# zhukovanadezhda/collaborative-filtering

Measured on AMD Instinct MI355X. Metric: ratings/sec per ALS iteration at k=64, higher is better.
Workload: dtype f32 (storage, solve, accumulate); Gram products as 2-way fp16 split (error <= 2^-23) on fp16 MFMA; rows over the condition limit redone in f64 (solve_dtype=auto)

## Files before the change

### collaborative-filtering_amd/csrc/als_device.hpp

```cpp
#pragma once
#include <hip/hip_runtime.h>
#include <stdint.h>
#include <type_traits>

typedef float f32x4 __attribute__((ext_vector_type(4)));
typedef float f32x2 __attribute__((ext_vector_type(2)));

#define ALS_EPS 1e-10f

__device__ __forceinline__ float readlane_f(float v, int src_lane) {
    return __int_as_float(__builtin_amdgcn_readlane(__float_as_int(v), src_lane));
}
__device__ __forceinline__ float bperm_f(float v, int src_lane) {
    return __int_as_float(__builtin_amdgcn_ds_bpermute(src_lane << 2, __float_as_int(v)));
}
__device__ __forceinline__ int bperm_i(int v, int src_lane) {
    return __builtin_amdgcn_ds_bpermute(src_lane << 2, v);
}
template <unsigned long long MASK>
__device__ __forceinline__ float select_lanes(float a, float b) {
    return __builtin_amdgcn_inverse_ballot_w64(MASK) ? a : b;
}
template <int BOUND, int RR>
constexpr unsigned long long lanes_below() {
    constexpr int n = BOUND - 64 * RR;
    return n <= 0 ? 0ull : (n >= 64 ? ~0ull : ((1ull << n) - 1ull));
}

__device__ __forceinline__ float wave_sum(float v) {
    auto dpp = [](float x, auto ctrl, auto rows) {
        return __int_as_float(__builtin_amdgcn_update_dpp(0, __float_as_int(x), decltype(ctrl)::value,
                                                          decltype(rows)::value, 0xf, false));
    };
    using std::integral_constant;
    v += dpp(v, integral_constant<int, 0xB1>{}, integral_constant<int, 0xf>{});
    v += dpp(v, integral_constant<int, 0x4E>{}, integral_constant<int, 0xf>{});
    v += dpp(v, integral_constant<int, 0x141>{}, integral_constant<int, 0xf>{});
    v += dpp(v, integral_constant<int, 0x140>{}, integral_constant<int, 0xf>{});
    v += dpp(v, integral_constant<int, 0x142>{}, integral_constant<int, 0xa>{});
    v += dpp(v, integral_constant<int, 0x143>{}, integral_constant<int, 0xc>{});
    return readlane_f(v, 63);
}
__device__ __forceinline__ float wave_max_nonneg(float v) {
    auto dpp = [](uint32_t x, auto ctrl, auto rows) {
        return (uint32_t)__builtin_amdgcn_update_dpp(0, (int)x, decltype(ctrl)::value, decltype(rows)::value, 0xf, false);
    };
    using std::integral_constant;
    uint32_t u = (uint32_t)__float_as_int(v);
    u = max(u, dpp(u, integral_constant<int, 0xB1>{}, integral_constant<int, 0xf>{}));
    u = max(u, dpp(u, integral_constant<int, 0x4E>{}, integral_constant<int, 0xf>{}));
    u = max(u, dpp(u, integral_constant<int, 0x141>{}, integral_constant<int, 0xf>{}));
    u = max(u, dpp(u, integral_constant<int, 0x140>{}, integral_constant<int, 0xf>{}));
    u = max(u, dpp(u, integral_constant<int, 0x142>{}, integral_constant<int, 0xa>{}));
    u = max(u, dpp(u, integral_constant<int, 0x143>{}, integral_constant<int, 0xc>{}));
    return __int_as_float(__builtin_amdgcn_readlane((int)u, 63));
}
__device__ __forceinline__ double wave_sum_d(double v) {
#pragma unroll
    for (int o = 32; o >= 1; o >>= 1) v += __shfl_xor(v, o, 64);
    return v;
}

__device__ __forceinline__ void wave_lds_sync() {
    __builtin_amdgcn_fence(__ATOMIC_SEQ_CST, "workgroup");
    __builtin_amdgcn_wave_barrier();
}

template <int KB>
__device__ __forceinline__ int perm_to_col(int p) { return KB * (p & 15) + (p >> 4); }

template <int KB>
__device__ __forceinline__ void load_frow(const float* __restrict__ p, float (&f)[KB]) {
    if constexpr (KB % 4 == 0) {
#pragma unroll
        for (int j = 0; j < KB / 4; ++j) {
            f32x4 v = *reinterpret_cast<const f32x4*>(p + 4 * j);
            f[4 * j] = v.x; f[4 * j + 1] = v.y; f[4 * j + 2] = v.z; f[4 * j + 3] = v.w;
        }
    } else if constexpr (KB % 2 == 0) {
#pragma unroll
        for (int j = 0; j < KB / 2; ++j) {
            f32x2 v = *reinterpret_cast<const f32x2*>(p + 2 * j);
            f[2 * j] = v.x; f[2 * j + 1] = v.y;
        }
    } else {
#pragma unroll
        for (int j = 0; j < KB; ++j) f[j] = p[j];
    }
}

template <int KB>
struct KCfg {
    static constexpr int KP = 16 * KB;
    static constexpr int NACC = KB * (KB + 1) / 2;
    static constexpr int NR = (KP + 63) / 64;
    static constexpr int lcol_off(int J) { return 16 * (J * KP - 8 * J * (J - 1)); }
    __device__ static __forceinline__ int lcol_off_rt(int J) { return 16 * (J * KP - 8 * J * (J - 1)); }
    static constexpr int LDS_FLOATS = lcol_off(KB);
    static_assert(lcol_off(KB) == NACC * 256, "the L image and a full accumulator set have the same size");
#ifndef ALS_WPW
#define ALS_WPW 1
#endif
    static constexpr int WPW = ALS_WPW;
#ifndef ALS_MINW_LE4
#define ALS_MINW_LE4 3
#endif
    static constexpr int MINW = (KB <= 4) ? ALS_MINW_LE4 : (KB <= 6 ? 2 : 1);
    static constexpr int SLOT_ITEMS = NACC * 4 + 2 * KB + 2;
    static constexpr int GS = (KB <= 8) ? 8 : 4;
};

template <int KP>
__device__ __forceinline__ float solve_regs(const float (&a)[KP], float di, float rb, int lane,
                                            float* y_out = nullptr) {
    int zero;
    asm volatile("s_mov_b32 %0, 0" : "=s"(zero));
    const unsigned long long ones = ~0ull;
    float rs = rb * di;
#pragma unroll
    for (int j = 0; j < KP; ++j) {
        const float yj = readlane_f(rs, j);
        const unsigned long long mask = (j >= 63) ? 0ull : (ones << (j + 1 + zero));
        const float cf = __builtin_amdgcn_inverse_ballot_w64(mask) ? a[j] * di : 0.f;
        rs = fmaf(-cf, yj, rs);
    }
    if (y_out) *y_out = rs;
    rs *= di;
#pragma unroll
    for (int i = KP - 1; i >= 0; --i) {
        const float xi = readlane_f(rs, i);
        const unsigned long long mask = (i <= 0) ? 0ull : ~(ones << (i + zero));
        const float cf = __builtin_amdgcn_inverse_ballot_w64(mask) ? a[i] * di : 0.f;
        rs = fmaf(-cf, xi, rs);
    }
    return rs;
}

template <int KB>
__device__ __forceinline__ void solve_stream_plain(const float* __restrict__ M, float (&rb)[KCfg<KB>::NR], int lane,
                                             float* y_out = nullptr) {
    constexpr int KP = KCfg<KB>::KP, NR = KCfg<KB>::NR;
    int ic[NR];
    float di[NR], rs[NR];
#pragma unroll
    for (int rr = 0; rr < NR; ++rr) {
        ic[rr] = min(lane + 64 * rr, KP - 1);
        di[rr] = M[ic[rr] * KP + ic[rr]];
        rs[rr] = rb[rr] * di[rr];
// ... 331 lines not shown
```

### collaborative-filtering_amd/csrc/gs_sweep.hip

```cpp
#include <atomic>
#include <cstdlib>
#include "als_device.hpp"
#include "als_hip.h"

extern "C" int als_gs_sweep(const als_gs_sweep_params* p, void* stream);

namespace {

template <int KB>
struct GsCfg {
    static constexpr int WPW = (KB <= 4) ? 4 : (KB <= 6 ? 2 : 1);
};

template <int KB>
__global__ __launch_bounds__(64 * GsCfg<KB>::WPW)
void k_gs_level(const als_gs_sweep_params P) {
    using C = KCfg<KB>;
    constexpr int KP = C::KP, NR = C::NR;
    constexpr int LD = KP + 1;
    constexpr int IMG = KP * LD + 3 * KP;
    __shared__ float lds_all[(KB <= 4) ? 1 : GsCfg<KB>::WPW * IMG];
    const int lane = threadIdx.x & 63;
    const int wave = threadIdx.x >> 6;
    const int64_t tid = (int64_t)blockIdx.x * GsCfg<KB>::WPW + wave;
// ... 128 lines not shown
    const int64_t i64 = item;
    const int64_t s0 = P.S_ptr[item], s1 = P.S_ptr[item + 1];
    const double* M = (const double*)P.factor + i64 * KP * KP;
    const double* rhs = (const double*)P.rhs + i64 * KP;
    const double* colsum = (const double*)P.colsum + i64 * KP;
    int ic[NR], col[NR];
    double g[NR];
#pragma unroll
    for (int rr = 0; rr < NR; ++rr) {
        ic[rr] = min(lane + 64 * rr, KP - 1);
        col[rr] = perm_to_col<KB>(ic[rr]);
        g[rr] = 0.0;
    }
    for (int64_t t = s0; t < s1; ++t) {
        const int sj = P.S_idx[t];
        const double sv = (double)P.S_val[t];
#pragma unroll
        for (int rr = 0; rr < NR; ++rr) g[rr] = fma(sv, (double)P.V[(int64_t)sj * P.ld + col[rr]], g[rr]);
    }
    double di[NR], rs[NR], rhs_i[NR], y[NR];
#pragma unroll
    for (int rr = 0; rr < NR; ++rr) {
        di[rr] = M[ic[rr] * KP + ic[rr]];
        rhs_i[rr] = rhs[ic[rr]];
        rs[rr] = (rhs_i[rr] + (double)P.alpha * g[rr]) * di[rr];
    }
    for (int j = 0; j < KP; ++j) {
        double sel = rs[0];
#pragma unroll
        for (int rr = 1; rr < NR; ++rr) sel = ((j >> 6) == rr) ? rs[rr] : sel;
        const double yj = readlane_f64(sel, j & 63);
#pragma unroll
        for (int rr = 0; rr < NR; ++rr) {
            const double cf = (lane + 64 * rr > j) ? M[j * KP + ic[rr]] * di[rr] : 0.0;
            rs[rr] = fma(-cf, yj, rs[rr]);
        }
    }
#pragma unroll
    for (int rr = 0; rr < NR; ++rr) { y[rr] = rs[rr]; rs[rr] *= di[rr]; }
    for (int i = KP - 1; i >= 0; --i) {
        double sel = rs[0];
#pragma unroll
        for (int rr = 1; rr < NR; ++rr) sel = ((i >> 6) == rr) ? rs[rr] : sel;
        const double xi = readlane_f64(sel, i & 63);
#pragma unroll
        for (int rr = 0; rr < NR; ++rr) {
            const double cf = (lane + 64 * rr < i) ? M[i * KP + ic[rr]] * di[rr] : 0.0;
            rs[rr] = fma(-cf, xi, rs[rr]);
        }
    }
    double dot = 0.0, xr = 0.0, yy = 0.0, xx = 0.0;
#pragma unroll
    for (int rr = 0; rr < NR; ++rr)
        if (lane + 64 * rr < KP) {
            const double x = rs[rr];
            P.V[i64 * P.ld + col[rr]] = (float)x;
            dot = fma(colsum[ic[rr]], x, dot); xr = fma(rhs_i[rr], x, xr);
            yy = fma(y[rr], y[rr], yy); xx = fma(x, x, xx);
        }
    dot = wave_sum_d(dot);
    const double nnz = (double)(P.indptr[item + 1] - P.indptr[item]);
    const double lb = (double)(P.lambda_bias_row ? P.lambda_bias_row[item] : P.lambda_bias_scalar);
    const double sumr = ((const double*)P.sumr)[item];
    const double bnew = (sumr - dot) / (nnz + lb + 1e-10);
    const double bold = (double)P.bias[item];
    __builtin_amdgcn_sched_barrier(0);
    if (lane == 0) P.bias[item] = (float)bnew;
    if (P.stat_out) {
        xr = wave_sum_d(xr); yy = wave_sum_d(yy); xx = wave_sum_d(xx);
        if (lane == 0) {
            const double sumr2 = ((const double*)P.sumr2)[item];
            const double s1v = sumr - nnz * bnew;
            const double s2v = sumr2 - 2.0 * bnew * sumr + nnz * bnew * bnew;
            const double cross = xr + (bold - bnew) * dot;
            const double quad = yy - (double)P.lambda_eff[item] * xx;
            P.stat_out[2 * i64] = (float)(s1v - dot);
            P.stat_out[2 * i64 + 1] = (float)(s2v - 2.0 * cross + quad);
        }
    }
}

constexpr unsigned GS_SENTINEL = 0x7fc0dea1u;

__device__ __forceinline__ float ld_agent(const float* p) {
    return __int_as_float(__hip_atomic_load(reinterpret_cast<const int*>(p), __ATOMIC_RELAXED, __HIP_MEMORY_SCOPE_AGENT));
}
__device__ __forceinline__ void st_agent(float* p, float v) {
    __hip_atomic_store(reinterpret_cast<int*>(p), __float_as_int(v), __ATOMIC_RELAXED, __HIP_MEMORY_SCOPE_AGENT);
}

#ifdef ALS_GS_STAMPS
__device__ unsigned long long g_gs_stamps[8];
#define GS_STAMP(slot) do { const unsigned long long now_ = __builtin_amdgcn_s_memtime(); st_acc[slot] += now_ - st_t; st_t = now_; } while (0)
#else
#define GS_STAMP(slot) do { } while (0)
#endif

template <int KB, bool STREAM>
struct DfCfg {
    static constexpr bool IMAGE = KB > 4 && !STREAM;
    static constexpr int WPW = IMAGE ? 1 : 4;
    static constexpr int LD = KCfg<KB>::KP + 1;
    static constexpr int IMG = IMAGE ? KCfg<KB>::KP * LD + 3 * KCfg<KB>::KP : 1;
};

template <int KB, bool STREAM>
__global__ __launch_bounds__((64 * DfCfg<KB, STREAM>::WPW), (DfCfg<KB, STREAM>::IMAGE ? 1 : 2))
void k_gs_dataflow(const als_gs_sweep_params P, const int32_t* __restrict__ Sw, float* pub,
                   int32_t* err, int64_t nitems, int nwaves, const float* __restrict__ nondep) {
    using C = KCfg<KB>;
    constexpr int KP = C::KP, NR = C::NR;
    using D = DfCfg<KB, STREAM>;
    constexpr int LD = D::LD;
    constexpr bool IMAGE = D::IMAGE;
    constexpr unsigned long long SPIN_LIMIT = 1ull << 27;
    __shared__ float lds_img[D::IMG];
    float* Al = lds_img;
    float* vec = lds_img + (IMAGE ? KP * LD : 0);
    float* dinv = vec + (IMAGE ? 2 * KP : 0);
    const int lane = threadIdx.x & 63;
    const int gw = blockIdx.x * D::WPW + (threadIdx.x >> 6);
    int ic[NR], col[NR];
#pragma unroll
    for (int rr = 0; rr < NR; ++rr) {
        ic[rr] = min(lane + 64 * rr, KP - 1);
        col[rr] = perm_to_col<KB>(ic[rr]);
    }
#ifdef ALS_GS_STAMPS
    unsigned long long st_acc[6] = {0, 0, 0, 0, 0, 0};
    unsigned long long st_t = __builtin_amdgcn_s_memtime();
#endif
    for (int64_t it = gw; it < nitems; it += nwaves) {
        const int item = P.items[it];
        const int64_t i64 = item;
        const int64_t s0 = P.S_ptr[item], s1 = P.S_ptr[item + 1];
        const float nnz = (float)(P.indptr[item + 1] - P.indptr[item]);
        const float lb = P.lambda_bias_row ? P.lambda_bias_row[item] : P.lambda_bias_scalar;
        const float* M = P.factor + i64 * KP * KP;
        constexpr int KPR = (KB <= 4) ? KP : 1;
        float a[KPR];
        float di0 = 0.f;
        if constexpr (KB <= 4) {
#pragma unroll
            for (int p = 0; p < KP; ++p) a[p] = M[p * KP + ic[0]];
            di0 = M[ic[0] * KP + ic[0]];
        } else if constexpr (IMAGE) {
            for (int p0 = 0; p0 < KP; p0 += 8) {
                float t[8][NR];
#pragma unroll
                for (int u = 0; u < 8; ++u)
#pragma unroll
                    for (int rr = 0; rr < NR; ++rr) t[u][rr] = M[(p0 + u) * KP + ic[rr]];
#pragma unroll
                for (int u = 0; u < 8; ++u)
#pragma unroll
                    for (int rr = 0; rr < NR; ++rr)
                        if (lane + 64 * rr < KP) {
                            Al[(p0 + u) * LD + ic[rr]] = t[u][rr];
                            if (ic[rr] == p0 + u) dinv[ic[rr]] = t[u][rr];
                        }
            }
        }
        float rhs_i[NR], cs_i[NR], g[NR];
#pragma unroll
        for (int rr = 0; rr < NR; ++rr) {
            rhs_i[rr] = P.rhs[i64 * KP + ic[rr]];
            cs_i[rr] = P.colsum[i64 * KP + ic[rr]];
            g[rr] = 0.f;
        }
        constexpr int GB = (NR == 1) ? 16 : 8;
#ifdef ALS_GS_STAMPS
        asm volatile("s_waitcnt vmcnt(0)" ::: "memory");
// ... 366 lines not shown
```

### collaborative-filtering_amd/csrc/row_solve.hip

```cpp
#include <type_traits>
#include "als_device.hpp"
#include "als_hip.h"
#include "row_common.hpp"

namespace {

template <int KB>
struct RowAcc {
    f32x4 acc[KCfg<KB>::NACC];
    float rhs[KB];
    float cs[KB];
    float sumr;
    float sumr2;
    __device__ __forceinline__ void zero() {
#pragma unroll
        for (int a = 0; a < KCfg<KB>::NACC; ++a) acc[a] = f32x4{0.f, 0.f, 0.f, 0.f};
#pragma unroll
        for (int b = 0; b < KB; ++b) { rhs[b] = 0.f; cs[b] = 0.f; }
        sumr = 0.f; sumr2 = 0.f;
    }
};

template <int KB, bool FULL>
__device__ __forceinline__ void process_chunk(RowAcc<KB>& A, int off_l, float r_l, int nvalid,
// ... 181 lines not shown
    const int c = lane & 15, q = lane >> 4;
    const float* Fc = F + KB * c;
    int nflush = 0;
    f32x4 E[MODE == 2 ? KB : 1];
    const uint32_t* Pc = planes + KB * c;
    const int sel_c = (c == 0) ? 0x05040100 : (c == 2) ? 0x07060302 : 0x0c0c0c0c;
    const int ones_c = (c == 1) ? 0x3C003C00 : 0;
    const float inv_s = __int_as_float((254 - ((__float_as_int(S) >> 23) & 0xff)) << 23);
    if constexpr (MODE == 2) {
#pragma unroll
        for (int b = 0; b < KB; ++b) E[b] = f32x4{0.f, 0.f, 0.f, 0.f};
    }
    int idx1 = (lane < len) ? __builtin_nontemporal_load(idxp + lane) : zero_row;
    int idx2 = (64 + lane < len) ? __builtin_nontemporal_load(idxp + 64 + lane) : zero_row;
    float val1 = (lane < len) ? __builtin_nontemporal_load(valp + lane) : 0.f;
    float bo1 = (lane < len) ? bias_other[idx1] : 0.f;
    for (int base = 0; base < len; base += 64) {
        const int idx0 = idx1;
        const float val0 = val1, bo0 = bo1;
        idx1 = idx2;
        const int t2 = base + 128 + lane;
        idx2 = (t2 < len) ? __builtin_nontemporal_load(idxp + t2) : zero_row;
        const int t1 = base + 64 + lane;
        val1 = (t1 < len) ? __builtin_nontemporal_load(valp + t1) : 0.f;
        bo1 = (t1 < len) ? bias_other[idx1] : 0.f;
        const int nvalid = min(64, len - base);
        const bool ok = lane < nvalid;
        const float rb = val0 - mu - bo0;
        A.sumr += ok ? rb : 0.f;
        A.sumr2 = ok ? fmaf(rb, rb, A.sumr2) : A.sumr2;
        const float r0 = ok ? (rb - bself) : 0.f;
        const int off0 = idx0 * ld;
        if constexpr (MODE == 0) {
            if (nvalid == 64) process_chunk<KB, true>(A, off0, r0, 64, Fc, q);
            else              process_chunk<KB, false>(A, off0, r0, nvalid, Fc, q);
        } else {
            if constexpr (MODE == 2) {
                const _Float16 rh = (_Float16)r0;
                const _Float16 rl = (_Float16)(r0 - (float)rh);
                const int rp = (int)__builtin_bit_cast(unsigned short, rh) | ((int)__builtin_bit_cast(unsigned short, rl) << 16);
                if (nvalid == 64) process_chunk_planes<KB, true>(A, E, off0, rp, 64, Pc, q, sel_c, ones_c);
                else              process_chunk_planes<KB, false>(A, E, off0, rp, nvalid, Pc, q, sel_c, ones_c);
            } else {
                if (nvalid == 64) process_chunk_f16x2<KB, true>(A, off0, r0, 64, Fc, q, S);
                else              process_chunk_f16x2<KB, false>(A, off0, r0, nvalid, Fc, q, S);
            }
            if (((base >> 6) + 1) % (FLUSH_GROUPS / 2) == 0 && base + 64 < len) {
                mfma_results_settle();
                if constexpr (MODE == 2) fold_planes_rhs<KB>(A, E, q, inv_s);
                flush_acc<KB>(A, Ls, lane, nflush == 0);
                ++nflush;
            }
        }
    }
    if (MODE != 0) mfma_results_settle();
    if constexpr (MODE == 2) fold_planes_rhs<KB>(A, E, q, inv_s);
    if (MODE != 0 && nflush > 0) {
        unflush_acc<KB>(A, Ls, lane);
        wave_lds_sync();
    }
}

template <int KB>
__device__ __forceinline__ void store_partial(const RowAcc<KB>& A, float* __restrict__ ws, int lane) {
    int it = 0;
#pragma unroll
    for (int a = 0; a < KCfg<KB>::NACC; ++a)
#pragma unroll
        for (int r = 0; r < 4; ++r) ws[(it++) * 64 + lane] = A.acc[a][r];
#pragma unroll
    for (int b = 0; b < KB; ++b) ws[(it++) * 64 + lane] = A.rhs[b];
#pragma unroll
    for (int b = 0; b < KB; ++b) ws[(it++) * 64 + lane] = A.cs[b];
    ws[(it++) * 64 + lane] = A.sumr;
    ws[it * 64 + lane] = A.sumr2;
}

template <int KB>
__device__ __forceinline__ void add_partial(RowAcc<KB>& A, const float* __restrict__ ws, int lane) {
    int it = 0;
#pragma unroll
    for (int a = 0; a < KCfg<KB>::NACC; ++a)
#pragma unroll
        for (int r = 0; r < 4; ++r) A.acc[a][r] += ws[(it++) * 64 + lane];
#pragma unroll
    for (int b = 0; b < KB; ++b) A.rhs[b] += ws[(it++) * 64 + lane];
#pragma unroll
    for (int b = 0; b < KB; ++b) A.cs[b] += ws[(it++) * 64 + lane];
    A.sumr += ws[(it++) * 64 + lane];
    A.sumr2 += ws[it * 64 + lane];
}

template <int KB, int J, int T, bool SOLVE>
__device__ __forceinline__ void panel_pivot(float (&p)[KCfg<KB>::NR][16], Chol<KB>& S, int lane) {
    constexpr int NR = KCfg<KB>::NR;
    constexpr int PIV = 16 * J + T, RP = PIV >> 6, LP = PIV & 63;
    constexpr int DR = (16 * J) >> 6, DL = (16 * J) & 63;
    const float prep = bperm_f(p[DR][T], DL + (lane & 15));
    const float d = readlane_f(p[RP][T], LP);
    const float inv = __builtin_amdgcn_rsqf(d);
    float l[NR];
#pragma unroll
    for (int rr = 0; rr < NR; ++rr) { l[rr] = p[rr][T] * inv; p[rr][T] = l[rr]; }
    float lrep = -(prep * inv);
    asm("s_nop 1" : "+v"(lrep));
    float yt = 0.f;
    if constexpr (SOLVE) yt = readlane_f(S.b[RP], LP) * inv;
    panel_trailing<KB, T + 1>(p, l, lrep);
    if constexpr (SOLVE) {
#pragma unroll
        for (int rr = 0; rr < NR; ++rr) S.b[rr] = fmaf(-l[rr], yt, S.b[rr]);
        S.y[RP] = select_lanes<1ull << LP>(yt, S.y[RP]);
    }
}

template <int KB, int J, int T, bool SOLVE>
__device__ __forceinline__ void panel_pivots(float (&p)[KCfg<KB>::NR][16], Chol<KB>& S, int lane) {
    if constexpr (T < 16) {
        panel_pivot<KB, J, T, SOLVE>(p, S, lane);
        panel_pivots<KB, J, T + 1, SOLVE>(p, S, lane);
    }
}

template <int KB, int J, bool SOLVE>
__device__ __forceinline__ void chol_panel(RowAcc<KB>& A, Chol<KB>& S, float* __restrict__ Ls, int lane) {
    using C = KCfg<KB>;
    constexpr int KP = C::KP, NR = C::NR;
    constexpr int OFF = C::lcol_off(J);
    const int c = lane & 15, q = lane >> 4;
    {
        const int swzc = (((c >> 2) ^ q) << 2) + (c & 3);
#pragma unroll
        for (int I = J; I < KB; ++I)
#pragma unroll
            for (int r = 0; r < 4; ++r)
                Ls[OFF + (16 * (I - J) + 4 * q + r) * 16 + swzc] = A.acc[blk_idx(I, J)][r];
    }
    wave_lds_sync();
    float p[NR][16];
    const int si = (lane >> 2) & 3;
#pragma unroll
    for (int rr = 0; rr < NR; ++rr) {
        const int i = lane + 64 * rr;
        const int rowi = min(max(i, 16 * J), KP - 1) - 16 * J;
#pragma unroll
        for (int g = 0; g < 4; ++g) {
            const f32x4 v = *reinterpret_cast<const f32x4*>(Ls + OFF + rowi * 16 + ((g ^ si) << 2));
            p[rr][4 * g] = v.x; p[rr][4 * g + 1] = v.y; p[rr][4 * g + 2] = v.z; p[rr][4 * g + 3] = v.w;
        }
    }
    wave_lds_sync();
    panel_pivots<KB, J, 0, SOLVE>(p, S, lane);
#pragma unroll
    for (int rr = 0; rr < NR; ++rr) {
        const int i = lane + 64 * rr;
        if (i >= 16 * J && i < KP) {
#pragma unroll
            for (int g = 0; g < 4; ++g) {
                const f32x4 v = {p[rr][4 * g], p[rr][4 * g + 1], p[rr][4 * g + 2], p[rr][4 * g + 3]};
                *reinterpret_cast<f32x4*>(Ls + OFF + (i - 16 * J) * 16 + ((g ^ si) << 2)) = v;
            }
        }
    }
    wave_lds_sync();
    {
        constexpr int DR = (16 * J) >> 6, DL = (16 * J) & 63;
        const float dl = Ls[OFF + c * 16 + (c & 3)];
        S.di[DR] = select_lanes<0xFFFFull << DL>(__builtin_amdgcn_rcpf(dl), S.di[DR]);
    }
    if constexpr (J + 1 < KB) {
        f32x4 op[KB - J - 1];
        const int sg = ((q ^ ((c >> 2) & 3)) << 2);
#pragma unroll
// ... 170 lines not shown
        chol_panels<KB, 0, true>(A, S, Ls, lane);
        const bool spd = chol_spd<KB>(S, lane);
        if (P.cond_limit > 0.f) {
            if (row_needs_f64<KB>(S, P, row, spd, mean_eig, short_row_bound, lane)) return;
        } else if (!spd && lane == 0) atomicMax(P.status, row + 1);
    }
    float x[NR];
    if (!(P.reserved0 & 4)) backward_solve<KB>(Ls, S, x, lane);
    else {
#pragma unroll
        for (int rr = 0; rr < NR; ++rr) x[rr] = S.y[rr];
    }

    float dot = 0.f, xr = 0.f, yy = 0.f, xx = 0.f;
#pragma unroll
    for (int rr = 0; rr < NR; ++rr) {
        if (lane + 64 * rr < KP) {
            dot = fmaf(csrow[rr], x[rr], dot);
            xr = fmaf(rhs0[rr], x[rr], xr);
            yy = fmaf(S.y[rr], S.y[rr], yy);
            xx = fmaf(x[rr], x[rr], xx);
        }
    }
    dot = wave_sum(dot);
    const float nnz = (float)(P.indptr[row + 1] - P.indptr[row]);
    const float lb = P.lambda_bias_row ? P.lambda_bias_row[row] : P.lambda_bias_scalar;
    const float bnew = (sumr - dot) / (nnz + lb + ALS_EPS);
    const float bold = P.bias_self[row];
    float st1 = 0.f, st2 = 0.f;
    if (P.stat_out) {
        xr = wave_sum(xr); yy = wave_sum(yy); xx = wave_sum(xx);
        const double bn = bnew, dt = dot;
        const double s1 = (double)sumr - (double)nnz * bn;
        const double s2 = (double)sumr2 - 2.0 * bn * (double)sumr + (double)nnz * bn * bn;
        const double cross = (double)xr + ((double)bold - bn) * dt;
        const double quad = (double)yy - (double)lam * (double)xx;
        const double sd2 = s2 - 2.0 * cross + quad;
        if (P.cond_limit > 0.f && !(sd2 >= 1e-3 * s2)) {
            if (lane == 0) P.redo_rows[atomicAdd(P.redo_count, 1)] = row;
            return;
        }
        st1 = (float)(s1 - dt);
        st2 = (float)sd2;
    }
#pragma unroll
    for (int rr = 0; rr < NR; ++rr)
        if (lane + 64 * rr < KP) P.X_out[r64 * P.ld + colrow[rr]] = x[rr];
    __builtin_amdgcn_sched_barrier(0);
    if (lane == 0) {
        P.bias_out[row] = bnew;
        if (P.stat_out) { P.stat_out[2 * r64] = st1; P.stat_out[2 * r64 + 1] = st2; }
    }
}

template <int KB, int MODE>
__global__ __launch_bounds__(64 * KCfg<KB>::WPW, KCfg<KB>::MINW)
void k_row_tasks(const als_row_solve_params P) {
    using C = KCfg<KB>;
    __shared__ __attribute__((aligned(16))) float lds_all[C::WPW * C::LDS_FLOATS];
    const int lane = threadIdx.x & 63;
    const int wave = threadIdx.x >> 6;
    const int wave_u = wave;
    const int64_t tid = (int64_t)blockIdx.x * C::WPW + wave_u;
    if (tid >= P.ntasks) return;
    const als_task t = P.tasks[tid];
    const int row = t.row;
    const int seg = t.seg;
    const int slot = t.slot;
    const int64_t rbeg = P.indptr[row], rend = P.indptr[row + 1];
    const int64_t beg = rbeg + (int64_t)seg * ALS_SPLIT_CHUNK;
    const int len = (int)min((int64_t)ALS_SPLIT_CHUNK, rend - beg);
    const float mu = (float)(*P.mu);
    const float bself = P.bias_self[row];

    const float S = (MODE != 0) ? P.F_scale[0] : 1.f;

    RowAcc<KB> A;
    A.zero();
    if (!(P.reserved0 & 1))
        gram_accumulate<KB, MODE>(A, P.indices + beg, P.vals + beg, len, P.F, P.ld, P.F_zero_row,
                                  P.bias_other, mu, bself, lane, lds_all + wave * C::LDS_FLOATS, S,
                                  (const uint32_t*)P.F_planes);
    if (slot >= 0) {
        store_partial<KB>(A, (float*)P.workspace + (size_t)slot * C::SLOT_ITEMS * 64, lane);
        return;
    }
    finish_row<KB>(A, P, row, lds_all + wave_u * C::LDS_FLOATS, lane);
}

template <int KB, int NB>
__device__ __forceinline__ void row_dual(const als_row_solve_params& P, int row, int64_t beg, int len,
                                         float* __restrict__ Ls, int lane) {
    constexpr int KP = KCfg<KB>::KP, NR = KCfg<KB>::NR, NSLAB = (KP + 31) / 32;
    constexpr int NS = KCfg<NB>::NR;
    const int c = lane & 15, q = lane >> 4;
    const float bold = P.bias_self[row];
    const float mu = (float)*P.mu;
    bool ok[NS];
    int idx_l[NS];
    float r_l[NS];
#pragma unroll
    for (int ss = 0; ss < NS; ++ss) {
        const int t = lane + 64 * ss;
        ok[ss] = t < len;
        idx_l[ss] = ok[ss] ? P.indices[beg + t] : P.F_zero_row;
        r_l[ss] = ok[ss] ? (P.vals[beg + t] - mu - P.bias_other[idx_l[ss]]) - bold : 0.f;
    }
    const int nblk = (len + 15) >> 4;
    int off[NB];
#pragma unroll
    for (int I = 0; I < NB; ++I)
        off[I] = bperm_i(idx_l[(16 * I) >> 6], (16 * I + c) & 63) * P.ld;

    const float Sc = P.F_scale[0];
    RowAcc<NB> A;
    A.zero();
    for (int s = 0; s < NSLAB; ++s) {
        const bool in = 32 * s + 8 * q < KP;
        i32x4 H[NB], L[NB];
#pragma unroll
        for (int I = 0; I < NB; ++I) {
            float f[8];
            if (I < nblk && in) {
                const f32x4 v0 = *reinterpret_cast<const f32x4*>(P.F + (uint32_t)off[I] + 32 * s + 8 * q);
                const f32x4 v1 = *reinterpret_cast<const f32x4*>(P.F + (uint32_t)off[I] + 32 * s + 8 * q + 4);
                f[0] = v0.x; f[1] = v0.y; f[2] = v0.z; f[3] = v0.w; f[4] = v1.x; f[5] = v1.y; f[6] = v1.z; f[7] = v1.w;
            } else {
#pragma unroll
                for (int e = 0; e < 8; ++e) f[e] = 0.f;
            }
#pragma unroll
            for (int e = 0; e < 8; e += 2) {
                int hw, lw;
                split2(f[e], f[e + 1], Sc, hw, lw);
                H[I][e >> 1] = hw; L[I][e >> 1] = lw;
            }
        }
#pragma unroll
        for (int bi = 0; bi < NB; ++bi)
#pragma unroll
            for (int bj = 0; bj <= bi; ++bj) {
                if (bi >= nblk) continue;
                f32x4 acc = A.acc[blk_idx(bi, bj)];
                const h16x8 hi = __builtin_bit_cast(h16x8, H[bi]), hj = __builtin_bit_cast(h16x8, H[bj]);
                const h16x8 li = __builtin_bit_cast(h16x8, L[bi]), lj = __builtin_bit_cast(h16x8, L[bj]);
                acc = __builtin_amdgcn_mfma_f32_16x16x32_f16(li, hj, acc, 0, 0, 0);
                acc = __builtin_amdgcn_mfma_f32_16x16x32_f16(hi, lj, acc, 0, 0, 0);
                acc = __builtin_amdgcn_mfma_f32_16x16x32_f16(hi, hj, acc, 0, 0, 0);
                A.acc[blk_idx(bi, bj)] = acc;
            }
    }
    mfma_results_settle();
    {
        const float un = P.F_scale[1];
#pragma unroll
        for (int a = 0; a < KCfg<NB>::NACC; ++a) A.acc[a] *= un;
    }
    const float lam = (P.lambda_row ? P.lambda_row[row] : P.lambda_scalar) + ALS_EPS;
    const float dual_mean_eig = (P.cond_limit > 0.f) ? gram_trace<NB>(A, lane) / (float)max(min(len, P.k), 1) + lam : 0.f;
#pragma unroll
    for (int J = 0; J < NB; ++J) {
        const float dv = (16 * J + c < len) ? lam : 1.0f;
#pragma unroll
        for (int r = 0; r < 4; ++r) A.acc[blk_idx(J, J)][r] += (4 * q + r == c) ? dv : 0.f;
    }
    Chol<NB> S;
#pragma unroll
    for (int ss = 0; ss < NS; ++ss) { S.b[ss] = r_l[ss]; S.di[ss] = 0.f; S.y[ss] = 0.f; }
// ... 14 lines not shown
    for (int ss = 0; ss < NS; ++ss) {
        const int lim = min(len - 64 * ss, 64);
        for (int i0 = 0; i0 < lim; i0 += 8) {
            float fv[8][NR], wi[8];
#pragma unroll
            for (int u = 0; u < 8; ++u) {
                const int i = min(i0 + u, 63);
                wi[u] = (i0 + u < lim) ? readlane_f(w[ss], i) : 0.f;
                const int o = __builtin_amdgcn_readlane(idx_l[ss], i) * P.ld;
#pragma unroll
                for (int rr = 0; rr < NR; ++rr) fv[u][rr] = P.F[(uint32_t)o + min(lane + 64 * rr, KP - 1)];
            }
#pragma unroll
            for (int u = 0; u < 8; ++u)
#pragma unroll
                for (int rr = 0; rr < NR; ++rr) x[rr] = fmaf(fv[u][rr], wi[u], x[rr]);
        }
    }
    const int64_t r64 = row;
#pragma unroll
    for (int rr = 0; rr < NR; ++rr)
        if (lane + 64 * rr < KP) P.X_out[r64 * P.ld + lane + 64 * rr] = x[rr];
    const float nnz = (float)len;
    const float lb = P.lambda_bias_row ? P.lambda_bias_row[row] : P.lambda_bias_scalar;
    float wsum = 0.f;
#pragma unroll
    for (int ss = 0; ss < NS; ++ss) wsum += ok[ss] ? w[ss] : 0.f;
    const float sw = wave_sum(wsum);
    const float bnew = (nnz * bold + lam * sw) / (nnz + lb + ALS_EPS);
    if (lane == 0) P.bias_out[row] = bnew;
    if (P.stat_out) {
        float e1 = 0.f, e2 = 0.f;
#pragma unroll
        for (int ss = 0; ss < NS; ++ss) {
            const float e = ok[ss] ? (bold - bnew) + lam * w[ss] : 0.f;
            e1 += e;
            e2 = fmaf(e, e, e2);
        }
        const float s1 = wave_sum(e1), s2 = wave_sum(e2);
        if (lane == 0) { P.stat_out[2 * r64] = s1; P.stat_out[2 * r64 + 1] = s2; }
    }
}

template <int KB>
__global__ __launch_bounds__(256, 3)
void k_row_dual(const als_row_solve_params P, int64_t task0, int64_t ntail) {
    using C4 = KCfg<4>;
    __shared__ __attribute__((aligned(16))) float lds_all[4 * C4::LDS_FLOATS];
    const int lane = threadIdx.x & 63, wave = threadIdx.x >> 6;
    const int64_t tid = (int64_t)blockIdx.x * 4 + wave;
    if (tid >= ntail) return;
    float* Ls = lds_all + wave * C4::LDS_FLOATS;
    const int row = P.tasks[task0 + tid].row;
    const int64_t beg = P.indptr[row];
    const int len = (int)(P.indptr[row + 1] - beg);
    if (len > 64 || len < 1) {
        if (lane == 0) atomicMax(P.status, row + 1);
        return;
    }
    if (len <= 16) row_dual<KB, 1>(P, row, beg, len, Ls, lane);
    else if (len <= 32) row_dual<KB, 2>(P, row, beg, len, Ls, lane);
    else if (len <= 48) row_dual<KB, 3>(P, row, beg, len, Ls, lane);
    else row_dual<KB, 4>(P, row, beg, len, Ls, lane);
}

template <int KB>
__global__ __launch_bounds__(128, 2)
void k_row_dual_mid(const als_row_solve_params P, int64_t task0, int64_t nmid) {
    using C6 = KCfg<6>;
    __shared__ __attribute__((aligned(16))) float lds_all[2 * C6::LDS_FLOATS];
    const int lane = threadIdx.x & 63, wave = threadIdx.x >> 6;
    const int64_t tid = (int64_t)blockIdx.x * 2 + wave;
    if (tid >= nmid) return;
    float* Ls = lds_all + wave * C6::LDS_FLOATS;
    const int row = P.tasks[task0 + tid].row;
    const int64_t beg = P.indptr[row];
    const int len = (int)(P.indptr[row + 1] - beg);
    if (len > 96 || len <= 64) {
        if (lane == 0) atomicMax(P.status, row + 1);
        return;
    }
    if (len <= 80) row_dual<KB, 5>(P, row, beg, len, Ls, lane);
    else row_dual<KB, 6>(P, row, beg, len, Ls, lane);
}

template <int KB>
__global__ __launch_bounds__(64 * KCfg<KB>::WPW, KCfg<KB>::MINW)
void k_row_long(const als_row_solve_params P) {
    using C = KCfg<KB>;
    __shared__ __attribute__((aligned(16))) float lds_all[C::WPW * C::LDS_FLOATS];
    const int lane = threadIdx.x & 63;
    const int wave = threadIdx.x >> 6;
    const int64_t tid = (int64_t)blockIdx.x * C::WPW + wave;
    if (tid >= P.nlong) return;
    const als_long_row lr = P.long_rows[tid];
    RowAcc<KB> A;
    A.zero();
    add_partial<KB>(A, (const float*)P.workspace + (size_t)lr.slot0 * C::SLOT_ITEMS * 64, lane);
    finish_row<KB>(A, P, lr.row, lds_all + wave * C::LDS_FLOATS, lane);
}

template <int KB>
__global__ __launch_bounds__(256)
void k_sum_slots(const als_long_row* __restrict__ long_rows, float* __restrict__ workspace) {
    constexpr int N = KCfg<KB>::SLOT_ITEMS * 64;
    const als_long_row lr = long_rows[blockIdx.x];
    const int e = blockIdx.y * 256 + threadIdx.x;
    if (e >= N || lr.nslots < 2) return;
    float* w0 = workspace + (size_t)lr.slot0 * N + e;
    float acc = 0.f + w0[0];
    for (int s = 1; s < lr.nslots; ++s) acc += w0[(size_t)s * N];
    w0[0] = acc;
}

__global__ __launch_bounds__(256)
void k_factor_scale(const float* __restrict__ F, int64_t n4, float* __restrict__ scale, int32_t* __restrict__ redo_count) {
    __shared__ uint32_t wmax[4];
    const f32x4* __restrict__ F4 = reinterpret_cast<const f32x4*>(F);
    uint32_t m = 0;
    const int64_t stride = (int64_t)gridDim.x * 256;
    for (int64_t i = (int64_t)blockIdx.x * 256 + threadIdx.x; i < n4; i += 4 * stride) {
        f32x4 v[4];
#pragma unroll
        for (int u = 0; u < 4; ++u)
            v[u] = (i + u * stride < n4) ? F4[i + u * stride] : f32x4{0.f, 0.f, 0.f, 0.f};
#pragma unroll
        for (int u = 0; u < 4; ++u)
#pragma unroll
            for (int e = 0; e < 4; ++e) m = max(m, (uint32_t)__float_as_int(v[u][e]) & 0x7FFFFFFFu);
    }
#pragma unroll
    for (int o = 32; o >= 1; o >>= 1) m = max(m, (uint32_t)__shfl_xor((int)m, o, 64));
    if ((threadIdx.x & 63) == 0) wmax[threadIdx.x >> 6] = m;
    __syncthreads();
    if (threadIdx.x == 0) {
        uint32_t* w = reinterpret_cast<uint32_t*>(scale);
        atomicMax(&w[2], max(max(wmax[0], wmax[1]), max(wmax[2], wmax[3])));
        __threadfence();
        if (atomicAdd(&w[3], 1u) == gridDim.x - 1) {
            __threadfence();
            const uint32_t mx = atomicMax(&w[2], 0u);
            const int e = (int)(mx >> 23);
            const int se = min(max(268 - e, 67), 187);
            scale[0] = __int_as_float(se << 23);
            scale[1] = __int_as_float((381 - 2 * se) << 23);
            atomicExch(&w[2], 0u);
            atomicExch(&w[3], 0u);
            if (redo_count) *redo_count = 0;
        }
    }
}

int launch_factor_scale(const float* F, int64_t nfloats, float* scale, int32_t* redo_count, hipStream_t st) {
    const int64_t n4 = nfloats / 4;
    const unsigned grid = (unsigned)min((int64_t)512, max((int64_t)1, (n4 + 1023) / 1024));
    hipLaunchKernelGGL(k_factor_scale, dim3(grid), dim3(256), 0, st, F, n4, scale, redo_count);
    return hipGetLastError() == hipSuccess ? 0 : ALS_E_LAUNCH;
}

__global__ void k_reset_word(int32_t* w) { *w = 0; }

template <int KB>
__global__ __launch_bounds__(256)
void k_split_planes(const float* __restrict__ F, int64_t npieces, const float* __restrict__ scale,
                    uint32_t* __restrict__ planes) {
    typedef uint32_t u32x4 __attribute__((ext_vector_type(4)));
    const float S = scale[0];
    for (int64_t e = (int64_t)blockIdx.x * 256 + threadIdx.x; e < npieces; e += (int64_t)gridDim.x * 256) {
        uint32_t h[KB / 2], l[KB / 2];
#pragma unroll
        for (int v4 = 0; v4 < KB / 4; ++v4) {
            const f32x4 x = reinterpret_cast<const f32x4*>(F)[e * (KB / 4) + v4];
            int h01, l01, h23, l23;
            split2(x[0], x[1], S, h01, l01);
            split2(x[2], x[3], S, h23, l23);
            h[2 * v4] = (uint32_t)h01; h[2 * v4 + 1] = (uint32_t)h23;
            l[2 * v4] = (uint32_t)l01; l[2 * v4 + 1] = (uint32_t)l23;
        }
        if constexpr (KB == 4) {
            reinterpret_cast<u32x4*>(planes)[e] = u32x4{h[0], h[1], l[0], l[1]};
        } else {
            reinterpret_cast<u32x4*>(planes)[2 * e] = u32x4{h[0], h[1], h[2], h[3]};
            reinterpret_cast<u32x4*>(planes)[2 * e + 1] = u32x4{l[0], l[1], l[2], l[3]};
        }
    }
}

template <int KB>
int launch_row_solve(const als_row_solve_params* p, hipStream_t st) {
    using C = KCfg<KB>;
    const bool plain = p->gram_mode == ALS_GRAM_F16X2 && p->reserved0 == 0 && p->X_out && p->bias_out &&
                       !p->gram_out && !p->factor_out && !p->rhs_out && !p->colsum_out && !p->sumr_out &&
                       !p->sumr2_out && !p->rhs_extra && !p->diag_extra;
    int64_t ntail = 0, nmid = 0;
    if (plain && p->ndual_tail >= 0 && p->ndual_mid >= 0 && (int64_t)p->ndual_tail + p->ndual_mid <= p->ntasks) {
        ntail = p->ndual_tail;
        if constexpr (KB >= 7) nmid = p->ndual_mid;
    }
    const int64_t nprimal = p->ntasks - ntail - nmid;
    if (nprimal > 0) {
        als_row_solve_params q = *p;
        q.ntasks = nprimal;
        const unsigned grid = (unsigned)((nprimal + C::WPW - 1) / C::WPW);
        bool planes = false;
        if constexpr (KB == 4 || KB == 8)
            planes = p->gram_mode == ALS_GRAM_F16X2 && p->F_planes != nullptr && p->reserved0 == 0;
        if (planes) {
            if constexpr (KB == 4 || KB == 8) {
                const int64_t npieces = ((int64_t)p->F_zero_row + 1) * 16;
                const unsigned sgrid = (unsigned)min((int64_t)4096, (npieces + 255) / 256);
                hipLaunchKernelGGL(k_split_planes<KB>, dim3(sgrid), dim3(256), 0, st, p->F, npieces, p->F_scale,
                                   (uint32_t*)p->F_planes);
                hipLaunchKernelGGL((k_row_tasks<KB, 2>), dim3(grid), dim3(64 * C::WPW), 0, st, q);
            }
        } else if (p->gram_mode == ALS_GRAM_F16X2)
            hipLaunchKernelGGL((k_row_tasks<KB, 1>), dim3(grid), dim3(64 * C::WPW), 0, st, q);
        else
            hipLaunchKernelGGL((k_row_tasks<KB, 0>), dim3(grid), dim3(64 * C::WPW), 0, st, q);
    }
    {
        if (ntail > 0)
            hipLaunchKernelGGL(k_row_dual<KB>, dim3((unsigned)((ntail + 3) / 4)), dim3(256), 0, st, *p, nprimal + nmid, ntail);
    }
    if constexpr (KB >= 7) {
        if (nmid > 0)
            hipLaunchKernelGGL(k_row_dual_mid<KB>, dim3((unsigned)((nmid + 1) / 2)), dim3(128), 0, st, *p, nprimal, nmid);
    }
    if (p->nlong > 0) {
        hipLaunchKernelGGL(k_sum_slots<KB>, dim3((unsigned)p->nlong, (C::SLOT_ITEMS * 64 + 255) / 256), dim3(256), 0, st,
                           p->long_rows, (float*)p->workspace);
        const unsigned grid = (unsigned)((p->nlong + C::WPW - 1) / C::WPW);
        hipLaunchKernelGGL(k_row_long<KB>, dim3(grid), dim3(64 * C::WPW), 0, st, *p);
    }
    return hipGetLastError() == hipSuccess ? 0 : ALS_E_LAUNCH;
}

}

int als_row_solve_f64_dispatch(const als_row_solve_params* p, hipStream_t st);
int als_row_redo_f64_dispatch(const als_row_solve_params* p, hipStream_t st);

extern "C" int als_version(void) { return ALS_HIP_VERSION; }
extern "C" int als_padded_k(int k) { return (k < 1 || k > ALS_MAX_K) ? ALS_E_BADK : 16 * ((k + 15) / 16); }
extern "C" int als_perm_index(int k, int c) {
    const int ld = als_padded_k(k);
    if (ld < 0 || c < 0 || c >= ld) return ALS_E_BADARG;
    const int KB = ld / 16;
    return 16 * (c % KB) + c / KB;
}
extern "C" int64_t als_partial_slot_bytes(int k) {
    const int ld = als_padded_k(k);
    if (ld < 0) return ALS_E_BADK;
    const int KB = ld / 16;
    return (int64_t)(KB * (KB + 1) / 2 * 4 + 2 * KB + 2) * 64 * sizeof(float);
}

extern "C" int als_factor_scale(const float* F, int64_t nfloats, float* scale, void* stream) {
    if (!F || !scale || nfloats < 0 || (nfloats & 3) || ((uintptr_t)F & 15)) return ALS_E_BADARG;
    return launch_factor_scale(F, nfloats, scale, nullptr, (hipStream_t)stream);
}

extern "C" int als_row_solve(const als_row_solve_params* p, void* stream) {
    if (!p) return ALS_E_BADARG;
    const int ld = als_padded_k(p->k);
    if (ld < 0) return ALS_E_BADK;
    if (p->ld != ld || !p->indptr || !p->indices || !p->vals || !p->F || !p->bias_self ||
        !p->bias_other || !p->mu || !p->status || p->ntasks < 0 || p->nlong < 0 || p->F_zero_row < 0 ||
        (p->gram_mode != ALS_GRAM_F32 && p->gram_mode != ALS_GRAM_F16X2 && p->gram_mode != ALS_GRAM_F64) ||
        (int64_t)p->F_zero_row * ld >= ((int64_t)1 << 31))
        return ALS_E_BADARG;
    if (p->ntasks > 0 && !p->tasks) return ALS_E_BADARG;
    if (p->nlong > 0 && (!p->long_rows || !p->workspace)) return ALS_E_BADARG;
    if (p->factor_out) {
        if (!p->rhs_out || !p->colsum_out || !p->sumr_out) return ALS_E_BADARG;
    } else if (!p->X_out || !p->bias_out) {
        return ALS_E_BADARG;
    }
    hipStream_t st = (hipStream_t)stream;
    if (p->gram_mode == ALS_GRAM_F64) return als_row_solve_f64_dispatch(p, st);
    const bool redo = p->cond_limit > 0.f;
    if (redo && (!p->redo_count || !p->redo_rows)) return ALS_E_BADARG;
    bool counter_reset = false;
    if (p->gram_mode == ALS_GRAM_F16X2) {
        if (!p->F_scale) return ALS_E_BADARG;
        if (!p->F_scale_ready) {
            const int rc = launch_factor_scale(p->F, ((int64_t)p->F_zero_row + 1) * ld, p->F_scale,
                                               redo ? p->redo_count : nullptr, st);
            if (rc != 0) return rc;
            counter_reset = true;
        }
    }
    if (redo && !counter_reset) hipLaunchKernelGGL(k_reset_word, dim3(1), dim3(1), 0, st, p->redo_count);
    int rc = ALS_E_BADK;
#ifdef ALS_KB_ONLY
    if (ld / 16 == ALS_KB_ONLY) rc = launch_row_solve<ALS_KB_ONLY>(p, st);
#else
    switch (ld / 16) {
        case 1: rc = launch_row_solve<1>(p, st); break;
        case 2: rc = launch_row_solve<2>(p, st); break;
        case 3: rc = launch_row_solve<3>(p, st); break;
        case 4: rc = launch_row_solve<4>(p, st); break;
        case 5: rc = launch_row_solve<5>(p, st); break;
        case 6: rc = launch_row_solve<6>(p, st); break;
        case 7: rc = launch_row_solve<7>(p, st); break;
        case 8: rc = launch_row_solve<8>(p, st); break;
        case 9: rc = launch_row_solve<9>(p, st); break;
        case 10: rc = launch_row_solve<10>(p, st); break;
    }
#endif
    if (rc == 0 && redo) rc = als_row_redo_f64_dispatch(p, st);
    return rc;
}
```

### include/als_hip.h

```cpp
#ifndef ALS_HIP_H
#define ALS_HIP_H

#include <stddef.h>
#include <stdint.h>

#ifdef __cplusplus
extern "C" {
#endif

#define ALS_HIP_VERSION 103
#define ALS_NXCD 8

#define ALS_E_BADARG   (-1)
#define ALS_E_BADK     (-2)
#define ALS_E_LAUNCH   (-3)

#define ALS_GRAM_F32    0
#define ALS_GRAM_F16X2  1
#define ALS_GRAM_F64    2

#define ALS_MAX_K 160
#define ALS_SPLIT_CHUNK 4096

typedef struct als_task {
    int32_t row;
    int32_t seg;
    int32_t slot;
    int32_t reserved;
} als_task;

typedef struct als_long_row {
    int32_t row;
    int32_t slot0;
    int32_t nslots;
    int32_t reserved;
} als_long_row;

int als_version(void);
int als_padded_k(int k);
int als_perm_index(int k, int c);
int64_t als_partial_slot_bytes(int k);
int64_t als_partial_slot_bytes_f64(int k);

typedef struct als_row_solve_params {
    int32_t k;
    int32_t ld;
    int64_t nrows;
    int32_t F_zero_row;
    int32_t reserved0;
    int32_t gram_mode;
    int32_t ndual_tail;
    int32_t ndual_mid;
    int32_t F_scale_ready;
    const int64_t* indptr;
    const int32_t* indices;
    const float*   vals;
    const float*   F;
    const float*   bias_self;
    const float*   bias_other;
    const double*  mu;
    float          lambda_scalar;
    const float*   lambda_row;
    float          lambda_bias_scalar;
    const float*   lambda_bias_row;
    const float*   rhs_extra;
    const float*   diag_extra;
    float*         X_out;
    float*         bias_out;
    float*         gram_out;
    float*         factor_out;
    float*         rhs_out;
    float*         colsum_out;
    float*         sumr_out;
    float*         sumr2_out;
    float*         stat_out;
    int32_t*       status;
    const als_task*     tasks;      int64_t ntasks;
    const als_long_row* long_rows;  int64_t nlong;
    void*          workspace;
    float          cond_limit;
    int32_t        byproducts_f64;
    int32_t*       redo_count;
    int32_t*       redo_rows;
    float*         cond_out;
    float*         F_scale;
    void*          F_planes;
} als_row_solve_params;

int als_row_solve(const als_row_solve_params* p, void* stream);

#define ALS_FSCALE_FLOATS 4
int als_factor_scale(const float* F, int64_t nfloats, float* scale, void* stream);

typedef struct als_gs_sweep_params {
    int32_t k, ld;
    const int32_t* items;  int64_t nitems;
    const int64_t* S_ptr;  const int32_t* S_idx;  const float* S_val;
    float alpha;
    const float* factor;  const float* rhs;  const float* colsum;
    const float* sumr;
    const int64_t* indptr;
    float lambda_bias_scalar;  const float* lambda_bias_row;
    float* V;
    float* bias;
    const float* sumr2;
    const float* lambda_eff;
    float* stat_out;
    int32_t f64;
    int32_t reserved;
} als_gs_sweep_params;

int als_gs_sweep(const als_gs_sweep_params* p, void* stream);

int als_gs_sweep_dataflow(const als_gs_sweep_params* p, const int32_t* S_idx_wait, float* publish,
                          int64_t nrows, float* nondep, int32_t* err, void* stream);

int als_gs_sweep_levels(const als_gs_sweep_params* p, const int64_t* level_offsets ,
                        int64_t nlevels, void* stream);

int als_residual_stats(int k, int ld, const int64_t* indptr, const int32_t* indices,
                       const float* vals, const float* U, const float* Z,
                       const float* b_u, const float* b_i, const double* mu,
                       const als_task* tasks, int64_t ntasks,
                       double* partials, double* out, void* stream);

typedef struct als_w_params {
    int32_t k, ld;
    int32_t phase;
    int32_t nfeat;
    int64_t item_begin, item_end;
    const float* gram;
    const float* rhs;
    const float* colsum;
    const float* V;
    const float* b_new;
    const float* b_old;
    int32_t D;
    int32_t f64;
    const float* X;
    const int32_t* feat_off;
    const float* W;
    float* H;
    int64_t nrows_h;
    int32_t feat_index, feat_col0, feat_d, nchunks;
    double* partA;
    double* partB;
    double* A_out;
    double* B_out;
} als_w_params;

int als_w_normal_equations(const als_w_params* p, void* stream);

#define ALS_SPD_MAX_N 8128
size_t als_spd_solve_workspace_bytes(int64_t N);
int als_spd_solve_f64(int64_t N, const double* A, int64_t lda, const double* b, double diag_add,
                      double* x, void* workspace, int32_t* status, void* stream);

int als_item_stats(int k, int ld, int64_t item_begin, int64_t item_end, const float* gram,
                   const float* rhs, const float* colsum, const float* sumr, const float* sumr2,
                   const int64_t* indptr, const float* Z, const float* b_new, const float* b_old,
                   float* stat_out, void* stream);
// ... 152 lines not shown
```

Baseline: 8.927 billion.

## Finish split long rows in last-arriving segment wave instead of separate kernels

Long rows split into segments previously needed two extra launches: one kernel summed the partial slots and another finished the row. Now each segment wave stores its partial, finds its long-row entry by binary search, and increments an arrival counter with release/acquire fences. The last segment to arrive sums all partials with agent-scope loads and runs finish_row itself. This removes two launches and a full pass over the workspace, at the cost of atomics, fences and a serial reduction done by a single wave. It also relies on the arrived counter starting at zero and being reset after use.

```diff
diff --git a/collaborative-filtering_amd/csrc/als_device.hpp b/collaborative-filtering_amd/csrc/als_device.hpp
--- a/collaborative-filtering_amd/csrc/als_device.hpp
+++ b/collaborative-filtering_amd/csrc/als_device.hpp
@@ -64,6 +64,13 @@
 __device__ __forceinline__ void wave_lds_sync() {
     __builtin_amdgcn_fence(__ATOMIC_SEQ_CST, "workgroup");
     __builtin_amdgcn_wave_barrier();
+}
+
+__device__ __forceinline__ float ld_agent(const float* p) {
+    return __int_as_float(__hip_atomic_load(reinterpret_cast<const int*>(p), __ATOMIC_RELAXED, __HIP_MEMORY_SCOPE_AGENT));
+}
+__device__ __forceinline__ void st_agent(float* p, float v) {
+    __hip_atomic_store(reinterpret_cast<int*>(p), __float_as_int(v), __ATOMIC_RELAXED, __HIP_MEMORY_SCOPE_AGENT);
 }
 
 template <int KB>
diff --git a/collaborative-filtering_amd/csrc/gs_sweep.hip b/collaborative-filtering_amd/csrc/gs_sweep.hip
--- a/collaborative-filtering_amd/csrc/gs_sweep.hip
+++ b/collaborative-filtering_amd/csrc/gs_sweep.hip
@@ -234,12 +234,6 @@
 
 constexpr unsigned GS_SENTINEL = 0x7fc0dea1u;
 
-__device__ __forceinline__ float ld_agent(const float* p) {
-    return __int_as_float(__hip_atomic_load(reinterpret_cast<const int*>(p), __ATOMIC_RELAXED, __HIP_MEMORY_SCOPE_AGENT));
-}
-__device__ __forceinline__ void st_agent(float* p, float v) {
-    __hip_atomic_store(reinterpret_cast<int*>(p), __float_as_int(v), __ATOMIC_RELAXED, __HIP_MEMORY_SCOPE_AGENT);
-}
 
 #ifdef ALS_GS_STAMPS
 __device__ unsigned long long g_gs_stamps[8];
diff --git a/collaborative-filtering_amd/csrc/row_solve.hip b/collaborative-filtering_amd/csrc/row_solve.hip
--- a/collaborative-filtering_amd/csrc/row_solve.hip
+++ b/collaborative-filtering_amd/csrc/row_solve.hip
@@ -287,13 +287,37 @@
 #pragma unroll
     for (int a = 0; a < KCfg<KB>::NACC; ++a)
 #pragma unroll
-        for (int r = 0; r < 4; ++r) A.acc[a][r] += ws[(it++) * 64 + lane];
-#pragma unroll
-    for (int b = 0; b < KB; ++b) A.rhs[b] += ws[(it++) * 64 + lane];
-#pragma unroll
-    for (int b = 0; b < KB; ++b) A.cs[b] += ws[(it++) * 64 + lane];
-    A.sumr += ws[(it++) * 64 + lane];
-    A.sumr2 += ws[it * 64 + lane];
+        for (int r = 0; r < 4; ++r) A.acc[a][r] += ld_agent(ws + (it++) * 64 + lane);
+#pragma unroll
+    for (int b = 0; b < KB; ++b) A.rhs[b] += ld_agent(ws + (it++) * 64 + lane);
+#pragma unroll
+    for (int b = 0; b < KB; ++b) A.cs[b] += ld_agent(ws + (it++) * 64 + lane);
+    A.sumr += ld_agent(ws + (it++) * 64 + lane);
+    A.sumr2 += ld_agent(ws + it * 64 + lane);
+}
+
+__device__ __forceinline__ bool segment_arrives_last(const als_row_solve_params& P, int row, int slot0, int nseg,
+                                                     int lane) {
+    int64_t lo = 0, hi = P.nlong - 1;
+    while (lo < hi) {
+        const int64_t mid = (lo + hi + 1) >> 1;
+        if (P.long_rows[mid].slot0 <= slot0) lo = mid; else hi = mid - 1;
+    }
+    if (P.nlong < 1 || P.long_rows[lo].slot0 != slot0 || P.long_rows[lo].row != row || P.long_rows[lo].nslots != nseg) {
+        if (lane == 0) atomicMax(P.status, row + 1);
+        return false;
+    }
+    int32_t* cnt = &P.long_rows[lo].arrived;
+    asm volatile("s_waitcnt vmcnt(0)" ::: "memory");
+    __builtin_amdgcn_fence(__ATOMIC_RELEASE, "agent");
+    asm volatile("s_waitcnt vmcnt(0)" ::: "memory");
+    int prev = 0;
+    if (lane == 0) prev = __hip_atomic_fetch_add(cnt, 1, __ATOMIC_RELAXED, __HIP_MEMORY_SCOPE_AGENT);
+    prev = __builtin_amdgcn_readfirstlane(prev);
+    if (prev != nseg - 1) return false;
+    __builtin_amdgcn_fence(__ATOMIC_ACQUIRE, "agent");
+    if (lane == 0) __hip_atomic_store(cnt, 0, __ATOMIC_RELAXED, __HIP_MEMORY_SCOPE_AGENT);
+    return true;
 }
 
 template <int KB, int J, int T, bool SOLVE>
@@ -630,8 +654,19 @@
                                   P.bias_other, mu, bself, lane, lds_all + wave * C::LDS_FLOATS, S,
                                   (const uint32_t*)P.F_planes);
     if (slot >= 0) {
-        store_partial<KB>(A, (float*)P.workspace + (size_t)slot * C::SLOT_ITEMS * 64, lane);
-        return;
+        constexpr size_t SLOT = (size_t)C::SLOT_ITEMS * 64;
+        __builtin_amdgcn_sched_barrier(0);
+        int lane_s = lane;
+        asm volatile("" : "+v"(lane_s));
+        store_partial<KB>(A, (float*)P.workspace + (size_t)slot * SLOT, lane_s);
+        const int row_s = __builtin_amdgcn_readfirstlane(row);
+        const int nseg = (int)((P.indptr[row_s + 1] - P.indptr[row_s] + ALS_SPLIT_CHUNK - 1) / ALS_SPLIT_CHUNK);
+        const int64_t tid_s = (int64_t)blockIdx.x * C::WPW + __builtin_amdgcn_readfirstlane(threadIdx.x >> 6);
+        const int slot0 = __builtin_amdgcn_readfirstlane(slot) - P.tasks[tid_s].seg;
+        if (!segment_arrives_last(P, row_s, slot0, nseg, lane_s)) return;
+        A.zero();
+#pragma unroll 1
+        for (int s = 0; s < nseg; ++s) add_partial<KB>(A, (const float*)P.workspace + (size_t)(slot0 + s) * SLOT, lane_s);
     }
     finish_row<KB>(A, P, row, lds_all + wave_u * C::LDS_FLOATS, lane);
 }
@@ -812,35 +847,6 @@
     }
     if (len <= 80) row_dual<KB, 5>(P, row, beg, len, Ls, lane);
     else row_dual<KB, 6>(P, row, beg, len, Ls, lane);
-}
-
-template <int KB>
-__global__ __launch_bounds__(64 * KCfg<KB>::WPW, KCfg<KB>::MINW)
-void k_row_long(const als_row_solve_params P) {
-    using C = KCfg<KB>;
-    __shared__ __attribute__((aligned(16))) float lds_all[C::WPW * C::LDS_FLOATS];
-    const int lane = threadIdx.x & 63;
-    const int wave = threadIdx.x >> 6;
-    const int64_t tid = (int64_t)blockIdx.x * C::WPW + wave;
-    if (tid >= P.nlong) return;
-    const als_long_row lr = P.long_rows[tid];
-    RowAcc<KB> A;
-    A.zero();
-    add_partial<KB>(A, (const float*)P.workspace + (size_t)lr.slot0 * C::SLOT_ITEMS * 64, lane);
-    finish_row<KB>(A, P, lr.row, lds_all + wave * C::LDS_FLOATS, lane);
-}
-
-template <int KB>
-__global__ __launch_bounds__(256)
-void k_sum_slots(const als_long_row* __restrict__ long_rows, float* __restrict__ workspace) {
-    constexpr int N = KCfg<KB>::SLOT_ITEMS * 64;
-    const als_long_row lr = long_rows[blockIdx.x];
-    const int e = blockIdx.y * 256 + threadIdx.x;
-    if (e >= N || lr.nslots < 2) return;
-    float* w0 = workspace + (size_t)lr.slot0 * N + e;
-    float acc = 0.f + w0[0];
-    for (int s = 1; s < lr.nslots; ++s) acc += w0[(size_t)s * N];
-    w0[0] = acc;
 }
 
 __global__ __launch_bounds__(256)
@@ -956,12 +962,6 @@
         if (nmid > 0)
             hipLaunchKernelGGL(k_row_dual_mid<KB>, dim3((unsigned)((nmid + 1) / 2)), dim3(128), 0, st, *p, nprimal, nmid);
     }
-    if (p->nlong > 0) {
-        hipLaunchKernelGGL(k_sum_slots<KB>, dim3((unsigned)p->nlong, (C::SLOT_ITEMS * 64 + 255) / 256), dim3(256), 0, st,
-                           p->long_rows, (float*)p->workspace);
-        const unsigned grid = (unsigned)((p->nlong + C::WPW - 1) / C::WPW);
-        hipLaunchKernelGGL(k_row_long<KB>, dim3(grid), dim3(64 * C::WPW), 0, st, *p);
-    }
     return hipGetLastError() == hipSuccess ? 0 : ALS_E_LAUNCH;
 }
 
diff --git a/include/als_hip.h b/include/als_hip.h
--- a/include/als_hip.h
+++ b/include/als_hip.h
@@ -33,7 +33,7 @@
     int32_t row;
     int32_t slot0;
     int32_t nslots;
-    int32_t reserved;
+    int32_t arrived;
 } als_long_row;
 
 int als_version(void);
@@ -76,7 +76,7 @@
     float*         stat_out;
     int32_t*       status;
     const als_task*     tasks;      int64_t ntasks;
-    const als_long_row* long_rows;  int64_t nlong;
+    als_long_row*       long_rows;  int64_t nlong;
     void*          workspace;
     float          cond_limit;
     int32_t        byproducts_f64;
```

Result: slower. 8.575 billion (-4.0%).
